# borisfoko/Spark-Text-Clustering

Measured on AMD Instinct MI355X. Metric: LDA E-step docs/sec (node) at k=100, V=2^18; % of HBM roofline, higher is better.
Workload: dtype f64

## Files before the change

### spark-text-clustering_amd/csrc/lda_rows64.hip

```cpp
#include "estep_common.h"
#include "psi64.h"
#include "rows64_layout.h"

#ifndef R64_LOAD_BATCH
#define R64_LOAD_BATCH 3
#endif
#ifndef R64_PRIO
#define R64_PRIO 2
#endif
#ifndef R64_RCP_NR
#define R64_RCP_NR 2
#endif
#ifndef R64_MIRROR
#define R64_MIRROR 1
#endif
#ifndef R64_SB_LDS
#define R64_SB_LDS 0
#endif
#ifndef R64_PSI_TPL
#define R64_PSI_TPL 1
#endif
#ifndef R64_SB_SWZ
#define R64_SB_SWZ 1
#endif
#ifndef R64_PA_LAYOUT
#define R64_PA_LAYOUT 1
#endif
#ifndef R64_LONG_OCC
#define R64_LONG_OCC 1
#endif

namespace stc {
namespace lda {

namespace {

constexpr int kW = 4;
using r64::kPaPitch;
using r64::kSbPitch;
constexpr int kOnChipSets = 6;
constexpr int kMaxSets = 8;

constexpr int kSxPitch = 10;

template <int KL_, int RREG_, int RMAX_>
struct RShape {
  static constexpr int KL = KL_;
  static constexpr int KLP = (KL_ + 1) / 2 * 2;
  static constexpr int KT = 8 * KL_;
  static constexpr int RREG = RREG_;
  static constexpr int RMAX = RMAX_;
  static constexpr int NOVF = RMAX_ > RREG_ ? RMAX_ - RREG_ : 0;
};
template <int KL>
using RCommon = RShape<KL, 5, kOnChipSets>;
template <int KL>
using RLong = RShape<KL, kMaxSets, kMaxSets>;

template <class S>
struct RLds {
  double eth[8][S::KLP] __attribute__((aligned(16)));
  double gam[S::KT];
  double rrow[kW][8 * S::RMAX];
  int rid[kW][8 * S::RMAX];
  double dsum[2];
  double esum[kW] __attribute__((aligned(16)));
  double part[kW][4];
  double cs;
  double apc[S::KT][2] __attribute__((aligned(16)));
  double ac[4] __attribute__((aligned(16)));
  PsiK psik;
  union {
    struct {
      union {
        double pa[8 * S::RMAX][kPaPitch];
        double sx[R64_SB_LDS ? S::KT * kSxPitch : 1] __attribute__((aligned(16)));
      } wv[kW];
      double sb[S::KT][kSbPitch];
    } l;
    double stage[kW][8][S::KT + 2];
  } u __attribute__((aligned(16)));
  double ovf[S::NOVF > 0 ? S::NOVF * kW * S::KL * 64 : 1];
};

struct RDoc {
  int64_t slot, row, mem, s0, e0;
  int nnz, rsets;
  int tid;
  int lane, w, tl, rl;
  int npsi, half, pw, tt, ttl, ttp;
  bool tval, town;
  bool wv;
  int qid;
  double qc, qls, qe2;
#ifdef STC_STAMP
  unsigned long long st0;
#endif
};

template <bool RES>
__device__ __forceinline__ int rows64_tid(const RDoc& d) { return RES ? d.tid : (int)threadIdx.x; }

template <class S, bool STATS, bool BOUND, bool RES, int NPSI>
__device__ __forceinline__ bool rows64_open(const EStepArgs<double>& a, RLds<S>& sm, RDoc& d) {
  const int tid = rows64_tid<RES>(d);
  constexpr int KL = S::KL, KLP = S::KLP;
  const int k = a.k, kp = a.kp;
  const int lane = tid & 63, w = __builtin_amdgcn_readfirstlane(tid >> 6);
  d.lane = lane;
  d.w = w;
  d.tl = lane & 7;
  d.rl = lane >> 3;
  d.npsi = NPSI ? NPSI : (kp > 64 ? 2 : 1);
  d.half = d.npsi == 2 ? (kp + 1) / 2 : kp;
  d.pw = d.npsi == 2 ? (w & 1) : 0;
  d.tt = d.pw * d.half + lane;
  d.tval = lane < d.half && d.tt < kp;
  d.town = lane < d.half && d.tt < k;
  d.ttl = d.tt / KL;
  d.ttp = d.tt - d.ttl * KL;
  const int npsi = d.npsi, tt = d.tt;

  const int qn = 32 * (lane >> 3) + 8 * w + (lane & 7);
  d.wv = lane < 8 * d.rsets && qn < d.nnz;
  const int64_t qe = d.wv ? d.s0 + qn : 0;
  d.qid = d.wv ? a.indices[qe] : 0;
  d.qc = d.wv ? a.values[qe] : 0.0;

  double g0 = 0.0;
  const double alp = d.town ? a.alpha[tt] : 0.0;
  const double pc = d.town ? a.psic[tt] : 0.0;
  if (w < npsi) {
    if (d.tval) {
      sm.apc[tt][0] = alp;
      sm.apc[tt][1] = pc;
    }
    if (d.town) {
      if (a.gamma0) {
        g0 = a.gamma0[d.mem * k + tt];
      } else {
        const uint64_t key = a.key_mode == 0 ? train_doc_key(a.iteration, a.rank, d.mem) : (uint64_t)(a.doc_id_base + d.row);
#ifdef R64_DIAG_NORNG
        g0 = 1.0 + 1e-3 * (double)(key & 1023) + 1e-4 * tt;
#else
        g0 = gamma_sample(doc_stream(a.seed, key), tt, a.gamma_shape);
#endif
      }
    }
    if (d.tval) sm.gam[tt] = g0;
  }
  for (int i = tid; i < 8 * KLP; i += 64 * kW) (&sm.eth[0][0])[i] = 0.0;
  psik_fill(sm.psik, tid, 64 * kW);
  {
    const double gs = wave_sum_d(g0), as = wave_sum_d(alp), cts = wave_sum_d(d.qc);
    if (lane == 0) {
      sm.part[w][0] = w < npsi ? gs : 0.0;
      sm.part[w][1] = w < npsi ? as : 0.0;
      sm.part[w][2] = cts;
    }
  }
  const bool nonempty = __syncthreads_or(d.wv && d.qc != 0.0) != 0;
  const double gsum0 = (sm.part[0][0] + sm.part[1][0]) + (sm.part[2][0] + sm.part[3][0]);
  if (tid == 0) {
    const double asum = (sm.part[0][1] + sm.part[1][1]) + (sm.part[2][1] + sm.part[3][1]);
    const double ctot = (sm.part[0][2] + sm.part[1][2]) + (sm.part[2][2] + sm.part[3][2]);
    sm.ac[0] = asum;
    sm.ac[1] = ctot;
    sm.ac[2] = digamma_fast_d(asum + ctot);
  }

  if (!nonempty) {
    if (w < npsi) {
      if (d.town) {
        if (a.gamma) a.gamma[d.mem * k + tt] = 0.0;
        if (STATS) a.elogth[d.slot * k + tt] = 0.0;
      }
      if (STATS && d.tval) a.eth[d.slot * kp + tt] = 0.0;
    }
    if (tid == 0) {
      if (a.iters) a.iters[d.mem] = 0;
      if (a.nonempty) a.nonempty[d.mem] = 0;
      if (BOUND) a.bound[d.mem] = 0.0;
    }
    return false;
  }
  {
    const double cs0 = digamma_fast_d(gsum0);
    if (w < npsi && d.town) sm.eth[d.ttl][d.ttp] = exp_digamma_minus_v2<R64_RCP_NR>(g0, cs0 + pc);
    if (tid == 0) sm.cs = cs0;
  }
  return true;
}

template <class S, int R, int NPSI>
__device__ __forceinline__ int rows64_iterate(const EStepArgs<double>& a, RLds<S>& sm, RDoc& d, double& qdt) {
  constexpr int KL = S::KL, KLP = S::KLP;
  static_assert(NPSI < 2 || S::KT > 64, "two ψ waves: kp > 64");
  constexpr int RG = R < S::RREG ? R : S::RREG;
  static_assert(R >= 1 && R <= S::RMAX && R - RG <= S::NOVF, "row sets");
  STAMP_DECL
#ifdef STC_STAMP
  st_acc[10] += st_last - d.st0;
#endif
  const int lane = d.lane, w = d.w, tl = d.tl, rl = d.rl;
  const int k = a.k, kp = a.kp, nnz = d.nnz, tt = d.tt, ttl = d.ttl, ttp = d.ttp;
  const int npsi = NPSI ? NPSI : d.npsi, pw = NPSI ? (NPSI == 2 ? (w & 1) : 0) : d.pw;
  const bool town = d.town;
  const int qid = d.qid;
  const double qc = d.qc;
  d.qls = a.logscale[qid];
  const bool mir = R64_MIRROR && npsi == 2;
  double gm = 0.0, em = 0.0;

  double B[RG][KL];
  double* const ovf = sm.ovf + (size_t)w * KL * 64 + lane;
#define BV(j, p) ((j) < RG ? B[(j) < RG ? (j) : 0][p] : ovf[((j) - RG) * kW * KL * 64 + 64 * (p)])
  {
    const int C2 = kp >> 1;
    constexpr int NP = (8 * (S::KT / 2) + 63) / 64;
    double* const stg = &sm.u.stage[w][0][0];
    constexpr int SP = S::KT + 2;
#pragma unroll
    for (int j0 = 0; j0 < R; j0 += R64_LOAD_BATCH) {
      double2 pc[R64_LOAD_BATCH][NP];
#pragma unroll
      for (int jj = 0; jj < R64_LOAD_BATCH; ++jj) {
        const int j = j0 + jj;
        if (j >= R) break;
#pragma unroll
        for (int i = 0; i < NP; ++i) {
          const int c = lane + 64 * i;
          const int srow = c / C2, q = c - srow * C2;
          const int id = __builtin_amdgcn_ds_bpermute((8 * j + (srow & 7)) << 2, qid);
          const bool keep = c < 8 * C2 && 32 * j + 8 * w + srow < nnz;
#ifdef R64_DIAG_NOGATHER
          const double2 x = make_double2(1e-3 * (id & 7), 1e-3 * (q & 7));
#else
          const double2 x = *reinterpret_cast<const double2*>(a.Bp + (int64_t)(keep ? id : 0) * kp + 2 * (keep ? q : 0));
#endif
          pc[jj][i] = keep ? x : make_double2(0.0, 0.0);
        }
      }
#pragma unroll
      for (int jj = 0; jj < R64_LOAD_BATCH; ++jj) {
        const int j = j0 + jj;
        if (j >= R) break;
#pragma unroll
        for (int i = 0; i < NP; ++i) {
          const int c = lane + 64 * i;
          const int srow = c / C2, q = c - srow * C2;
          if (c < 8 * C2) *reinterpret_cast<double2*>(stg + srow * SP + 2 * q) = pc[jj][i];
        }
        __builtin_amdgcn_wave_barrier();
#pragma unroll
        for (int p = 0; p < KL; ++p) {
          const int t = KL * tl + p;
          const double v = t < k ? stg[rl * SP + t] : 0.0;
          if (j < RG) B[j < RG ? j : 0][p] = v;
          else ovf[(j - RG) * kW * KL * 64 + 64 * p] = v;
        }
        __builtin_amdgcn_wave_barrier();
      }
    }
  }

  const double qe2 = d.wv ? fmin(0x1p53 * exp(kLogEps - d.qls), 1e300) : -0x1p53;
  d.qe2 = qe2;
  __syncthreads();
  if (mir && town) {
    gm = sm.gam[tt];
    em = sm.eth[ttl][ttp];
  }

  double* const pa = &sm.u.l.wv[w].pa[0][0];
  int paw_o = 8 * (r64::pa_row(rl, R64_PA_LAYOUT) + tl), par_o = 8 * r64::pa_row(lane, R64_PA_LAYOUT);
#if R64_PA_LAYOUT
  asm volatile("" : "+v"(paw_o), "+v"(par_o));
#endif
  double* const paw = reinterpret_cast<double*>(reinterpret_cast<char*>(pa) + paw_o);
  double* const sb = &sm.u.l.sb[0][0];
  int sbw_o = 8 * r64::sb_slot(KL, tl, 2 * rl, w, R64_SB_SWZ);
  int sp0_o = 8 * (tt * kSbPitch + 2 * r64::sb_read_first(tt, R64_SB_SWZ));
  int sp1_o = 8 * (tt * kSbPitch + 2 * (r64::sb_read_first(tt, R64_SB_SWZ) ^ 1));
#if R64_SB_SWZ
  asm volatile("" : "+v"(sbw_o), "+v"(sp0_o), "+v"(sp1_o));
#endif
  [[maybe_unused]] double* const sbw = reinterpret_cast<double*>(reinterpret_cast<char*>(sb) + sbw_o);
  const double2* const sp0 = reinterpret_cast<const double2*>(reinterpret_cast<const char*>(sb) + sp0_o);
  const double2* const sp1 = reinterpret_cast<const double2*>(reinterpret_cast<const char*>(sb) + sp1_o);
  double* const esw = &sm.esum[w];
  const PsiExpK expk = psi_expk_load(sm.psik);
  double rr[R];
  double qr = 0.0;
  qdt = 0.0;
  double dsum = 0.0;
  int it = 0;
  STAMP(0);
  while (true) {
    {
      double acc[R];
#pragma unroll
      for (int j = 0; j < R; ++j) acc[j] = 0.0;
      constexpr bool OVP = R64_SB_LDS != 0 && R > RG;
      constexpr int NO = OVP ? 2 * (R - RG) : 1;
      double2 en = make_double2(0.0, 0.0);
      double on[NO] = {};
      if constexpr (OVP) {
        en = *reinterpret_cast<const double2*>(&sm.eth[tl][0]);
#pragma unroll
        for (int j = RG; j < R; ++j) {
          on[2 * (j - RG)] = BV(j, 0);
          if (1 < KL) on[2 * (j - RG) + 1] = BV(j, 1);
        }
      }
#pragma unroll
      for (int c = 0; c < KLP / 2; ++c) {
        const double2 e = OVP ? en : *reinterpret_cast<const double2*>(&sm.eth[tl][2 * c]);
        double oc[NO];
#pragma unroll
        for (int i = 0; i < NO; ++i) oc[i] = on[i];
        if (OVP && c + 1 < KLP / 2) {
          en = *reinterpret_cast<const double2*>(&sm.eth[tl][2 * c + 2]);
#pragma unroll
          for (int j = RG; j < R; ++j) {
            on[2 * (j - RG)] = BV(j, 2 * c + 2 < KL ? 2 * c + 2 : 0);
            if (2 * c + 3 < KL) on[2 * (j - RG) + 1] = BV(j, 2 * c + 3 < KL ? 2 * c + 3 : 0);
          }
        }
#pragma unroll
        for (int j = 0; j < R; ++j) {
          const int jo = OVP && j >= RG ? 2 * (j - RG) : 0;
          acc[j] = fma(OVP && j >= RG ? oc[jo] : BV(j, 2 * c), e.x, acc[j]);
          if (2 * c + 1 < KL) acc[j] = fma(OVP && j >= RG ? oc[jo + 1] : BV(j, 2 * c + 1), e.y, acc[j]);
        }
        if (OVP) __builtin_amdgcn_sched_barrier(0);
      }
#pragma unroll
      for (int j = 0; j < R; ++j) paw[8 * kPaPitch * j] = acc[j];
    }
    STAMP(1);
    __builtin_amdgcn_wave_barrier();
    if (R64_PRIO >= 2) __builtin_amdgcn_s_setprio(3);
    if (lane < 8 * R) {
      const double2* const pr = reinterpret_cast<const double2*>(reinterpret_cast<const char*>(pa) + par_o);
      const double2 x0 = pr[0], x1 = pr[1], x2 = pr[2], x3 = pr[3];
      qdt = ((x0.x + x0.y) + (x1.x + x1.y)) + ((x2.x + x2.y) + (x3.x + x3.y));
      const double ph = fma(qe2, 0x1p-53, qdt);
      qr = qc * rcp_nr(ph);
      sm.rrow[w][lane] = qr;
    }
#if R64_PSI_TPL
    const bool live = qe2 >= fma(qe2, 0x1p-53, qdt);
#else
    bool live = false;
    if (lane < 8 * R) live = qe2 >= fma(qe2, 0x1p-53, qdt);
#endif
    if (__builtin_amdgcn_ballot_w64(live) != 0) {
      const double e = wave_sum_d(lane < 8 * R ? qr * (qe2 * 0x1p-53) : 0.0);
      if (lane == 0) *esw = e;
    } else if (lane == 0) {
      *esw = 0.0;
    }
    __builtin_amdgcn_wave_barrier();
#pragma unroll
    for (int j = 0; j < R; ++j) rr[j] = sm.rrow[w][8 * j + rl];
    if (R64_PRIO >= 2) __builtin_amdgcn_s_setprio(0);
    STAMP(2);
    if ((it > 0 && dsum <= a.stop_thr) || it >= a.max_iter) break;

#if R64_SB_LDS
    {
      double* const sx = &sm.u.l.wv[w].sx[0];
      double* const sxw = sx + KL * tl * kSxPitch + rl;
      double ov[R > RG ? R - RG : 1][KL];
#pragma unroll
      for (int j = RG; j < R; ++j) {
#pragma unroll
        for (int p = 0; p < KL; ++p) ov[j - RG][p] = BV(j, p);
      }
#pragma unroll
      for (int p = 0; p < KL; ++p) {
        double acc = 0.0;
#pragma unroll
        for (int j = 0; j < R; ++j) acc = fma(j < RG ? BV(j, p) : ov[j < RG ? 0 : j - RG][p], rr[j], acc);
        sxw[p * kSxPitch] = acc;
      }
      __builtin_amdgcn_wave_barrier();
#pragma unroll
      for (int h = (S::KT - 1) / 64; h >= 0; --h) {
        const int t = lane + 64 * h;
        if (S::KT >= 64 * (h + 1) || t < S::KT) {
          const double2* const xr = reinterpret_cast<const double2*>(sx + t * kSxPitch);
          const double2 x01 = xr[0], x23 = xr[1], x45 = xr[2], x67 = xr[3];
          sb[t * kSbPitch + w] = ((x01.x + x45.x) + (x23.x + x67.x)) + ((x01.y + x45.y) + (x23.y + x67.y));
        }
      }
    }
#else
    {
      double x[16];
#pragma unroll
      for (int p = 0; p < 16; ++p) {
        double acc = 0.0;
        if (p < KL) {
#pragma unroll
          for (int j = 0; j < R; ++j) acc = fma(BV(j, p < KL ? p : 0), rr[j], acc);
        }
        x[p] = acc;
      }
      double s0, s1;
      rs_rows8(x, lane, s0, s1);
      if (2 * rl < KL) sbw[0] = s0;
      if (2 * rl + 1 < KL) sbw[kSbPitch] = s1;
    }
#endif
    STAMP(3);
    __syncthreads();
    STAMP(4);
    const bool psi = npsi == 2 ? ((w >> 1) == (it & 1)) : (w == (it & 3));
    if (psi) {
      if (R64_PRIO >= 1) __builtin_amdgcn_s_setprio(3);
      double dg = 0.0;
      if (town) {
        const double2 x0 = *sp0, x1 = *sp1;
        const double g = mir ? gm : sm.gam[tt], eo = sm.eth[ttl][ttp];
        const double2 ap = *reinterpret_cast<const double2*>(&sm.apc[tt][0]);
        const double2 e01 = *reinterpret_cast<const double2*>(&sm.esum[0]);
        const double2 e23 = *reinterpret_cast<const double2*>(&sm.esum[2]);
        const double s = (x0.x + x0.y) + (x1.x + x1.y);
        const double et = (e01.x + e01.y) + (e23.x + e23.y);
        const double csn = et != 0.0 ? digamma_fast_d(sm.ac[0] + sm.ac[1] - et) : sm.ac[2];
        const double gn = fma(eo, s, ap.x);
        dg = fabs(gn - g);
        sm.gam[tt] = gn;
        const double en = exp_digamma_minus_v4<R64_RCP_NR>(gn, csn + ap.y, expk);
        sm.eth[ttl][ttp] = en;
        gm = gn;
        em = en;
        if (tt == 0) sm.cs = csn;
      }
      if (!mir) {
        const double d = wave_sum_d(dg);
        if (lane == 0) sm.dsum[pw] = d;
      }
      if (R64_PRIO >= 1) __builtin_amdgcn_s_setprio(0);
    } else if (mir) {
      double dg = 0.0;
      if (town) {
        const double al = sm.apc[tt][0];
        const double2 y0 = *sp0, y1 = *sp1;
        const double s = (y0.x + y0.y) + (y1.x + y1.y);
        const double gn = fma(em, s, al);
        dg = fabs(gn - gm);
        gm = gn;
      }
      const double d = wave_sum_d(dg);
      if (lane == 0) sm.dsum[pw] = d;
    }
    STAMP(psi ? 5 : 8);
    __syncthreads();
    dsum = npsi == 2 ? sm.dsum[0] + sm.dsum[1] : sm.dsum[0];
    STAMP(psi ? 6 : 9);
    ++it;
  }
#undef BV
  STAMP_FLUSH
  return it;
}

template <class S, bool STATS, bool BOUND, bool RES>
__device__ __forceinline__ void rows64_close(const EStepArgs<double>& a, RLds<S>& sm, const RDoc& d, int it, double qdt) {
  const int tid = rows64_tid<RES>(d);
  const int lane = d.lane, w = d.w;
  const int k = a.k, kp = a.kp, nnz = d.nnz, npsi = d.npsi, tt = d.tt, ttl = d.ttl, ttp = d.ttp;
  const bool town = d.town, tval = d.tval, wv = d.wv;
  const int64_t slot = d.slot, mem = d.mem, e0 = d.e0;
  const int qid = d.qid;
  const double qc = d.qc, qls = d.qls;
#ifdef STC_STAMP
  const unsigned long long st_close = stamp_now();
#endif
  const double gfin = (w < npsi && town) ? sm.gam[tt] : 0.0;
  {
    const double gs = wave_sum_d(gfin);
    double bt = 0.0, bc = 0.0;
    if (BOUND && wv && qc != 0.0) {
      bt = qc * (log(fmax(qdt, 0x1p-1074)) + qls);
      bc = qc;
    }
    if (BOUND) {
      bt = wave_sum_d(bt);
      bc = wave_sum_d(bc);
    }
    if (lane == 0) {
      sm.part[w][0] = w < npsi ? gs : 0.0;
      sm.part[w][1] = bt;
      sm.part[w][2] = bc;
    }
    if (wv) sm.rid[w][lane] = qid;
  }
  __syncthreads();
  const double gsum = (sm.part[0][0] + sm.part[1][0]) + (sm.part[2][0] + sm.part[3][0]);
  const double psisum = digamma_t<double>(gsum);
  double topic = 0.0;
  if (w < npsi) {
    if (town) {
      const double el = digamma_t<double>(gfin) - psisum;
      if (a.gamma) a.gamma[mem * k + tt] = gfin;
      if (STATS) a.elogth[slot * k + tt] = el;
      if (BOUND) {
        const double alp = sm.apc[tt][0];
        topic = (alp - gfin) * el + (lgamma(gfin) - lgamma(alp));
      }
    }
    if (STATS && tval) a.eth[slot * kp + tt] = sm.eth[ttl][ttp];
  }
  for (int n = tid; n < nnz; n += 64 * kW) {
    const int ws = (n >> 3) & 3, q = 8 * (n >> 5) + (n & 7);
    const double rv = sm.rrow[ws][q];
    a.r[e0 + n] = rv;
    if (STATS && a.keys) {
      a.keys[e0 + n] = (uint32_t)sm.rid[ws][q];
      a.vals[e0 + n] = entry_val<double>(slot, e0 + n, rv);
    }
  }
  if (tid == 0) {
    if (a.iters) a.iters[mem] = it;
    if (a.nonempty) a.nonempty[mem] = 1;
  }
  if (BOUND) {
    topic = wave_sum_d(topic);
    if (lane == 0) sm.part[w][3] = topic;
    __syncthreads();
    if (tid == 0) {
      double tok = 0.0, ctk = 0.0, tp = 0.0;
#pragma unroll
      for (int v = 0; v < kW; ++v) {
        tok += sm.part[v][1];
        ctk += sm.part[v][2];
        tp += sm.part[v][3];
      }
      const double elog_max = sm.cs - psisum;
      a.bound[mem] = tok + ctk * elog_max + tp + (lgamma(sm.ac[0]) - lgamma(gsum));
    }
  }
#ifdef STC_STAMP
  if (lane == 0) atomicAdd(&g_stamps[7], stamp_now() - st_close);
#endif
}

template <class S, bool STATS, bool BOUND, int NPSI, bool LONG, bool RES = LONG>
__device__ __forceinline__ void rows64_doc(const EStepArgs<double>& a, RLds<S>& sm, RDoc& d) {
  d.e0 = a.bptr ? a.bptr[d.slot] : d.s0;
  if (!rows64_open<S, STATS, BOUND, RES, NPSI>(a, sm, d)) return;
  double qdt = 0.0;
  int it;
  if constexpr (LONG) {
    it = d.rsets == 7 ? rows64_iterate<S, 7, NPSI>(a, sm, d, qdt) : rows64_iterate<S, 8, NPSI>(a, sm, d, qdt);
  } else {
    switch (d.rsets) {
      case 1: it = rows64_iterate<S, 1, NPSI>(a, sm, d, qdt); break;
      case 2: it = rows64_iterate<S, 2, NPSI>(a, sm, d, qdt); break;
      case 3: it = rows64_iterate<S, 3, NPSI>(a, sm, d, qdt); break;
      case 4: it = rows64_iterate<S, 4, NPSI>(a, sm, d, qdt); break;
      case 5: it = rows64_iterate<S, 5, NPSI>(a, sm, d, qdt); break;
      default: it = rows64_iterate<S, 6, NPSI>(a, sm, d, qdt); break;
    }
  }
  rows64_close<S, STATS, BOUND, RES>(a, sm, d, it, qdt);
}

template <class S, bool STATS, bool BOUND, int NPSI>
__global__ __launch_bounds__(64 * kW, 2) void k_estep_rows64(EStepArgs<double> a) {
  __shared__ RLds<S> sm;
  if ((int64_t)blockIdx.x >= a.n) return;
  RDoc d;
#ifdef STC_STAMP
  d.st0 = stamp_now();
#endif
  d.slot = a.slot0 + blockIdx.x;
  d.row = a.batch ? (int64_t)a.batch[d.slot] : d.slot;
  d.mem = a.orig ? (int64_t)a.orig[d.slot] : d.slot;
  d.s0 = a.indptr[d.row];
  d.nnz = (int)(a.indptr[d.row + 1] - d.s0);
  d.rsets = (d.nnz + 31) >> 5;
  if (d.rsets > kOnChipSets) return;
  rows64_doc<S, STATS, BOUND, NPSI, false>(a, sm, d);
}

template <class S, bool STATS, bool BOUND, int NPSI>
__global__ __launch_bounds__(64 * kW, 2) void k_estep_rows64_pers(EStepArgs<double> a, int32_t* ticket) {
  __shared__ RLds<S> sm;
  __shared__ int s_tk;
  if (threadIdx.x == 0) s_tk = atomicAdd(ticket, 1);
  __syncthreads();
  int cur = s_tk;
  while (cur < a.n) {
    __syncthreads();
    int nxt = 0;
    if (threadIdx.x == 0) nxt = atomicAdd(ticket, 1);
    RDoc d;
#ifdef STC_STAMP
    d.st0 = stamp_now();
#endif
    d.tid = threadIdx.x;
    asm volatile("" : "+v"(d.tid));
    d.slot = a.slot0 + cur;
    d.row = a.batch ? (int64_t)a.batch[d.slot] : d.slot;
    d.mem = a.orig ? (int64_t)a.orig[d.slot] : d.slot;
    d.s0 = a.indptr[d.row];
    d.nnz = (int)(a.indptr[d.row + 1] - d.s0);
    d.rsets = (d.nnz + 31) >> 5;
    if (d.rsets <= kOnChipSets) rows64_doc<S, STATS, BOUND, NPSI, false, true>(a, sm, d);
    if (threadIdx.x == 0) s_tk = nxt;
    __syncthreads();
    cur = s_tk;
  }
}

__global__ void k_rows64_long_list(EStepArgs<double> a) {
  const int64_t i = (int64_t)blockIdx.x * blockDim.x + threadIdx.x;
  if (i >= a.n) return;
  const int64_t slot = a.slot0 + i;
  const int64_t row = a.batch ? (int64_t)a.batch[slot] : slot;
  const int nnz = (int)(a.indptr[row + 1] - a.indptr[row]);
  if (nnz > 32 * kOnChipSets) a.long_list[1 + atomicAdd(&a.long_list[0], 1)] = (int32_t)i;
}

template <class S, bool STATS, bool BOUND, int NPSI>
__global__ __launch_bounds__(64 * kW, R64_LONG_OCC) void k_estep_rows64_long(EStepArgs<double> a) {
  __shared__ RLds<S> sm;
  const int cnt = a.long_list[0];
  for (int j = blockIdx.x; j < cnt; j += gridDim.x) {
    RDoc d;
#ifdef STC_STAMP
    d.st0 = stamp_now();
#endif
    d.tid = threadIdx.x;
    asm volatile("" : "+v"(d.tid));
    d.slot = a.slot0 + a.long_list[1 + j];
    d.row = a.batch ? (int64_t)a.batch[d.slot] : d.slot;
    d.mem = a.orig ? (int64_t)a.orig[d.slot] : d.slot;
    d.s0 = a.indptr[d.row];
    d.nnz = (int)(a.indptr[d.row + 1] - d.s0);
    d.rsets = (d.nnz + 31) >> 5;
    rows64_doc<S, STATS, BOUND, NPSI, true>(a, sm, d);
    __syncthreads();
  }
}

template <class S, int NPSI>
bool launch_persist(hipStream_t s, const EStepArgs<double>& a, bool stats, bool bound) {
  if (!a.long_list || bound) return false;
  int32_t* ticket = a.long_list + a.n + 1;
  auto go = [&](const void* kern) {
    int dev = 0, cus = 0, per_cu = 0;
    HIP_CHECK(hipGetDevice(&dev));
    HIP_CHECK(hipDeviceGetAttribute(&cus, hipDeviceAttributeMultiprocessorCount, dev));
    HIP_CHECK(hipOccupancyMaxActiveBlocksPerMultiprocessor(&per_cu, kern, 64 * kW, 0));
    if (per_cu < 1) return false;
    HIP_CHECK(hipMemsetAsync(ticket, 0, sizeof(int32_t), s));
    EStepArgs<double> aa = a;
    void* args[] = {&aa, &ticket};
    const int64_t blocks = std::max<int64_t>(1, std::min<int64_t>(a.n, (int64_t)per_cu * cus));
    HIP_CHECK(hipLaunchKernel(kern, dim3((unsigned)blocks), dim3(64 * kW), args, 0, s));
    return true;
  };
  if (stats) return go((const void*)k_estep_rows64_pers<S, true, false, NPSI>);
  return go((const void*)k_estep_rows64_pers<S, false, false, NPSI>);
}
template <class S, int NPSI>
void launch_common(hipStream_t s, const EStepArgs<double>& a, bool stats, bool bound) {
  if (launch_persist<S, NPSI>(s, a, stats, bound)) return;
  const dim3 grid((unsigned)a.n);
  const int threads = 64 * kW;
  if (stats) k_estep_rows64<S, true, false, NPSI><<<grid, threads, 0, s>>>(a);
  else if (bound) k_estep_rows64<S, false, true, NPSI><<<grid, threads, 0, s>>>(a);
  else k_estep_rows64<S, false, false, NPSI><<<grid, threads, 0, s>>>(a);
  KERNEL_CHECK();
}
template <class S, int NPSI>
void launch_long(hipStream_t s, const EStepArgs<double>& a, bool stats, bool bound) {
  if (!a.long_list) throw Error(STC_ERR_STATE, "fp64 rows E-step: no long-document list buffer");
  HIP_CHECK(hipMemsetAsync(a.long_list, 0, sizeof(int32_t), s));
  k_rows64_long_list<<<dim3((unsigned)((a.n + 255) / 256)), 256, 0, s>>>(a);
  KERNEL_CHECK();
  int dev = 0, cus = 0;
  HIP_CHECK(hipGetDevice(&dev));
  HIP_CHECK(hipDeviceGetAttribute(&cus, hipDeviceAttributeMultiprocessorCount, dev));
  const dim3 grid((unsigned)std::max<int64_t>(1, std::min<int64_t>(a.n, (int64_t)cus * R64_LONG_OCC)));
  const int threads = 64 * kW;
  if (stats) k_estep_rows64_long<S, true, false, NPSI><<<grid, threads, 0, s>>>(a);
  else if (bound) k_estep_rows64_long<S, false, true, NPSI><<<grid, threads, 0, s>>>(a);
  else k_estep_rows64_long<S, false, false, NPSI><<<grid, threads, 0, s>>>(a);
  KERNEL_CHECK();
}
template <int KL, int NPSI>
void launch_r(hipStream_t s, const EStepArgs<double>& a, bool stats, bool bound, bool long_docs) {
  if (long_docs) launch_long<RLong<KL>, NPSI>(s, a, stats, bound);
  launch_common<RCommon<KL>, NPSI>(s, a, stats, bound);
}

}

int rows64_row_cap(int k) { return k <= 104 ? 32 * kMaxSets : 0; }
int rows64_onchip_rows(int k) { return k <= 104 ? 32 * kOnChipSets : 0; }

void launch_estep_rows64(hipStream_t s, const EStepArgs<double>& a, bool stats, bool bound, bool long_docs) {
  if (a.n == 0) return;
  if (a.kp > 8 * 13 || a.kp < a.k || (a.kp & 1)) throw Error(STC_ERR_INVALID_ARG, "fp64 rows E-step: bad k / kp");
  constexpr int kOne = R64_PSI_TPL ? 1 : 0, kTwo = R64_PSI_TPL ? 2 : 0;
  if (a.k <= 32) launch_r<4, kOne>(s, a, stats, bound, long_docs);
  else if (a.k <= 56) launch_r<7, kOne>(s, a, stats, bound, long_docs);
  else if (kTwo == 0 || a.kp > 64) launch_r<13, kTwo>(s, a, stats, bound, long_docs);
  else launch_r<13, kOne>(s, a, stats, bound, long_docs);
}

STC_STAMP_READER(stc_debug_stamps_rows64)

}
}
```

### spark-text-clustering_amd/csrc/psi64.h

```cpp
#pragma once

#include "estep_common.h"

namespace stc {
namespace lda {
namespace psi64 {

__device__ __forceinline__ double fma_s(double a, double b, double c) {
  double d;
  asm("v_fma_f64 %0, %1, %2, %3" : "=v"(d) : "v"(a), "v"(b), "s"(c));
  return d;
}
__device__ __forceinline__ double fma_sb(double a, double b, double c) {
  double d;
  asm("v_fma_f64 %0, %1, %2, %3" : "=v"(d) : "v"(a), "s"(b), "v"(c));
  return d;
}
__device__ __forceinline__ double mul_s(double a, double b) {
  double d;
  asm("v_mul_f64 %0, %1, %2" : "=v"(d) : "v"(a), "s"(b));
  return d;
}
__device__ __forceinline__ double add_s(double a, double b) {
  double d;
  asm("v_add_f64 %0, %1, %2" : "=v"(d) : "v"(a), "s"(b));
  return d;
}
__device__ __forceinline__ double sub_s(double b, double a) {
  double d;
  asm("v_add_f64 %0, -%1, %2" : "=v"(d) : "v"(a), "s"(b));
  return d;
}
typedef float pkf2 __attribute__((ext_vector_type(2)));
__device__ __forceinline__ double trunc_fix_pk(double f6, double xs) {
  const double nb = floor(sub_s(5.0, xs)) + 1.0;
  const float rb = __builtin_amdgcn_rcpf((float)xs + (float)nb);
  const pkf2 u = {(float)f6, rb * rb};
  pkf2 a = u * (pkf2)(-12318.55039822477f) + (pkf2)(2372.137971404805f);
  a = a * u + (pkf2)(-260.94994774566294f);
  a = a * u + (pkf2)(26.284421368293753f);
  a = a * u + (pkf2)(-3.053401198888146f);
  const pkf2 u2 = u * u, u4 = u2 * u2, u8 = u4 * u4;
  const pkf2 e = (u8 * u) * a;
  return (double)(e.x - e.y);
}
template <int RCP_STEPS>
__device__ __forceinline__ double rcp_n(double q) {
  double r = __builtin_amdgcn_rcp(q);
#pragma unroll
  for (int i = 0; i < RCP_STEPS; ++i) r = fma(r, fma(-q, r, 1.0), r);
  return r;
}
template <int RCP_STEPS>
__device__ __forceinline__ double exp_digamma_minus_v2(double x, double cst) {
  const bool sh = x <= 5.0;
  const double xs = sh ? x : 1.0;
  const double u = xs * add_s(xs, 5.0);
  const double num = fma_s(add_s(mul_s(u, 3.0), 20.0), u, 24.0) * fma(xs, 2.0, 5.0);
  const double den = u * fma_s(add_s(u, 10.0), u, 24.0);
  const double iq = rcp_n<RCP_STEPS>(den);
  double c = num * iq;
  c = fma(fma(-den, c, num), iq, c);
  const double y = sh ? add_s(x, 6.0) : x;
  const double iy = rcp_n<RCP_STEPS>(y);
  const double f = iy * iy;
  double t = add_s(mul_s(f, 3617.0 / 8160.0), -1.0 / 12.0);
  t = fma_s(t, f, 691.0 / 32760.0);
  t = fma_s(t, f, -1.0 / 132.0);
  t = fma_s(t, f, 1.0 / 240.0);
  t = fma_s(t, f, -1.0 / 252.0);
  t = fma_s(t, f, 1.0 / 120.0);
  t = fma_s(t, f, -1.0 / 12.0) * f;
  const double shift = sh ? trunc_fix_pk(f, xs) - c : 0.0;
  const double z = (fma(-0.5, iy, shift) + t) - cst;
  const double n = __builtin_rint(mul_s(z, 1.4426950408889634));
  double r = fma_sb(n, -6.93147180369123816490e-01, z);
  r = fma_sb(n, -1.90821492927058770002e-10, r);
  const double r2 = r * r;
  double e = add_s(mul_s(r2, 1.0 / 479001600.0), 1.0 / 3628800.0);
  e = fma_s(e, r2, 1.0 / 40320.0);
  e = fma_s(e, r2, 1.0 / 720.0);
  e = fma_s(e, r2, 1.0 / 24.0);
  e = fma(e, r2, 0.5);
  e = fma(e, r2, 1.0);
  double o = add_s(mul_s(r2, 1.0 / 6227020800.0), 1.0 / 39916800.0);
  o = fma_s(o, r2, 1.0 / 362880.0);
  o = fma_s(o, r2, 1.0 / 5040.0);
  o = fma_s(o, r2, 1.0 / 120.0);
  o = fma_s(o, r2, 1.0 / 6.0);
  o = fma(o, r2, 1.0);
  const double ez = __builtin_ldexp(fma(r, o, e), (int)fmax(n, -1100.0));
  return y * ez;
}

enum PsiKSlot {
  PK_LOG2E, PK_LN2HI, PK_LN2LO,
  PK_E0, PK_E1, PK_E2, PK_E3, PK_E4,
  PK_O0, PK_O1, PK_O2, PK_O3, PK_O5,
  PK_O4,
  PK_N
};
struct alignas(16) PsiK {
  double k[(PK_N + 1) / 2 * 2];
};
__device__ __forceinline__ void psik_fill(PsiK& t, int tid, int nthr) {
  const double v[PK_N] = {1.4426950408889634, -6.93147180369123816490e-01, -1.90821492927058770002e-10,
                          1.0 / 479001600.0, 1.0 / 3628800.0, 1.0 / 40320.0, 1.0 / 720.0, 1.0 / 24.0,
                          1.0 / 6227020800.0, 1.0 / 39916800.0, 1.0 / 362880.0, 1.0 / 5040.0, 1.0 / 120.0,
                          1.0 / 6.0};
  for (int i = tid; i < PK_N; i += nthr) t.k[i] = v[i];
}
struct PsiExpK {
  double log2e, ln2hi, ln2lo, e0, e1, e2, e3, e4, o0, o1, o2, o3, o5, o4;
};
__device__ __forceinline__ PsiExpK psi_expk_load(const PsiK& T) {
  const double* K = T.k;
  PsiExpK c{K[PK_LOG2E], K[PK_LN2HI], K[PK_LN2LO], K[PK_E0], K[PK_E1], K[PK_E2], K[PK_E3], K[PK_E4],
            K[PK_O0],    K[PK_O1],    K[PK_O2],    K[PK_O3], K[PK_O5], K[PK_O4]};
  asm volatile("" : "+v"(c.log2e), "+v"(c.ln2hi), "+v"(c.ln2lo), "+v"(c.e0), "+v"(c.e1), "+v"(c.e2), "+v"(c.e3));
  asm volatile("" : "+v"(c.e4), "+v"(c.o0), "+v"(c.o1), "+v"(c.o2), "+v"(c.o3), "+v"(c.o5), "+v"(c.o4));
  return c;
}
__device__ __forceinline__ double exp_vk(double z, const PsiExpK& C) {
#pragma clang fp contract(off)
  const double n = __builtin_rint(z * C.log2e);
  double r = __builtin_fma(n, C.ln2hi, z);
  r = __builtin_fma(n, C.ln2lo, r);
  const double r2 = r * r;
  double e = r2 * C.e0 + C.e1;
  e = __builtin_fma(e, r2, C.e2);
  e = __builtin_fma(e, r2, C.e3);
  e = __builtin_fma(e, r2, C.e4);
  e = __builtin_fma(e, r2, 0.5);
  e = __builtin_fma(e, r2, 1.0);
  double o = r2 * C.o0 + C.o1;
  o = __builtin_fma(o, r2, C.o2);
  o = __builtin_fma(o, r2, C.o3);
  o = __builtin_fma(o, r2, C.o5);
  o = __builtin_fma(o, r2, C.o4);
  o = __builtin_fma(o, r2, 1.0);
  return __builtin_ldexp(__builtin_fma(r, o, e), (int)fmax(n, -1100.0));
}
template <int RCP_STEPS>
__device__ __forceinline__ double exp_digamma_minus_v4(double x, double cst, const PsiExpK& C) {
  const bool sh = x <= 5.0;
  const double xs = sh ? x : 1.0;
  const double u = xs * add_s(xs, 5.0);
  const double num = fma_s(add_s(mul_s(u, 3.0), 20.0), u, 24.0) * fma(xs, 2.0, 5.0);
  const double den = u * fma_s(add_s(u, 10.0), u, 24.0);
  const double iq = rcp_n<RCP_STEPS>(den);
  double c = num * iq;
  c = fma(fma(-den, c, num), iq, c);
  const double y = sh ? add_s(x, 6.0) : x;
  const double iy = rcp_n<RCP_STEPS>(y);
  const double f = iy * iy;
  double t = add_s(mul_s(f, 3617.0 / 8160.0), -1.0 / 12.0);
  t = fma_s(t, f, 691.0 / 32760.0);
  t = fma_s(t, f, -1.0 / 132.0);
  t = fma_s(t, f, 1.0 / 240.0);
  t = fma_s(t, f, -1.0 / 252.0);
  t = fma_s(t, f, 1.0 / 120.0);
  t = fma_s(t, f, -1.0 / 12.0) * f;
  const double shift = sh ? trunc_fix_pk(f, xs) - c : 0.0;
  const double z = (fma(-0.5, iy, shift) + t) - cst;
  return y * exp_vk(z, C);
}

}
using psi64::exp_digamma_minus_v2;
using psi64::PsiK;
using psi64::psik_fill;
using psi64::PsiExpK;
using psi64::psi_expk_load;
using psi64::exp_digamma_minus_v4;
}
}
```

Before: 1.824 million.

## Defer dsum read, reorder psi update ahead of esum, skip redundant esum stores

Reads the convergence sums from shared memory during the next matvec instead of right after the second barrier, which takes an LDS load off the post-barrier critical path. The psi update now computes the digamma part before reading esum, and moves the rare correction behind an unlikely branch. The esum write is skipped when it was already zero on the previous iteration. An eager mode hoists x+6 and trunc_fix inside the psi polynomial, and lane-0 tests are made opaque to the compiler. These reorderings raise register pressure and add branch logic to a tight per-iteration loop.

```diff
diff --git a/spark-text-clustering_amd/csrc/lda_rows64.hip b/spark-text-clustering_amd/csrc/lda_rows64.hip
--- a/spark-text-clustering_amd/csrc/lda_rows64.hip
+++ b/spark-text-clustering_amd/csrc/lda_rows64.hip
@@ -25,6 +25,18 @@
 #endif
 #ifndef R64_PA_LAYOUT
 #define R64_PA_LAYOUT 1
+#endif
+#ifndef R64_DSUM_LATE
+#define R64_DSUM_LATE 1
+#endif
+#ifndef R64_PSI_FIRST
+#define R64_PSI_FIRST 1
+#endif
+#ifndef R64_PSI_EAGER
+#define R64_PSI_EAGER 1
+#endif
+#ifndef R64_WORKER_LINE
+#define R64_WORKER_LINE 1
 #endif
 #ifndef R64_LONG_OCC
 #define R64_LONG_OCC 1
@@ -294,6 +306,8 @@
   double qr = 0.0;
   qdt = 0.0;
   double dsum = 0.0;
+  [[maybe_unused]] double ds0 = 0.0, ds1 = 0.0;
+  [[maybe_unused]] uint32_t esnz = 1;
   int it = 0;
   STAMP(0);
   while (true) {
@@ -335,12 +349,38 @@
         }
         if (OVP) __builtin_amdgcn_sched_barrier(0);
       }
+#if R64_DSUM_LATE
+      ds0 = sm.dsum[0];
+      if (npsi == 2) ds1 = sm.dsum[1];
+#endif
 #pragma unroll
       for (int j = 0; j < R; ++j) paw[8 * kPaPitch * j] = acc[j];
     }
     STAMP(1);
     __builtin_amdgcn_wave_barrier();
     if (R64_PRIO >= 2) __builtin_amdgcn_s_setprio(3);
+#if R64_WORKER_LINE
+    {
+      double ph = -1.0;
+      if (lane < 8 * R) {
+        const double2* const pr = reinterpret_cast<const double2*>(reinterpret_cast<const char*>(pa) + par_o);
+        const double2 x0 = pr[0], x1 = pr[1], x2 = pr[2], x3 = pr[3];
+        qdt = ((x0.x + x0.y) + (x1.x + x1.y)) + ((x2.x + x2.y) + (x3.x + x3.y));
+        ph = fma(qe2, 0x1p-53, qdt);
+        qr = qc * rcp_nr(ph);
+        sm.rrow[w][lane] = qr;
+      }
+      const uint64_t vm = __builtin_amdgcn_ballot_w64(qe2 >= ph);
+      if (__builtin_expect(((uint32_t)vm | (uint32_t)(vm >> 32) | esnz) != 0, 0)) {
+        double e = 0.0;
+        if (vm != 0) e = wave_sum_d(lane < 8 * R ? qr * (qe2 * 0x1p-53) : 0.0);
+        int l0 = lane;
+        asm volatile("" : "+v"(l0));
+        if (l0 == 0) *esw = e;
+        esnz = __builtin_amdgcn_readfirstlane(vm != 0);
+      }
+    }
+#else
     if (lane < 8 * R) {
       const double2* const pr = reinterpret_cast<const double2*>(reinterpret_cast<const char*>(pa) + par_o);
       const double2 x0 = pr[0], x1 = pr[1], x2 = pr[2], x3 = pr[3];
@@ -361,12 +401,18 @@
     } else if (lane == 0) {
       *esw = 0.0;
     }
+#endif
     __builtin_amdgcn_wave_barrier();
 #pragma unroll
     for (int j = 0; j < R; ++j) rr[j] = sm.rrow[w][8 * j + rl];
     if (R64_PRIO >= 2) __builtin_amdgcn_s_setprio(0);
     STAMP(2);
+#if R64_DSUM_LATE
+    dsum = npsi == 2 ? ds0 + ds1 : ds0;
+    if (((int)(it > 0) & (int)(dsum <= a.stop_thr)) | (int)(it >= a.max_iter)) break;
+#else
     if ((it > 0 && dsum <= a.stop_thr) || it >= a.max_iter) break;
+#endif
 
 #if R64_SB_LDS
     {
@@ -427,13 +473,28 @@
         const double2 ap = *reinterpret_cast<const double2*>(&sm.apc[tt][0]);
         const double2 e01 = *reinterpret_cast<const double2*>(&sm.esum[0]);
         const double2 e23 = *reinterpret_cast<const double2*>(&sm.esum[2]);
+#if R64_PSI_FIRST
+        const double cflat = sm.ac[2];
+        const double s = (x0.x + x0.y) + (x1.x + x1.y);
+        const double gn = fma(eo, s, ap.x);
+        dg = fabs(gn - g);
+        sm.gam[tt] = gn;
+        double y;
+        const double zt = psi_part_v4<R64_RCP_NR, R64_PSI_EAGER != 0>(gn, y);
+        __builtin_amdgcn_sched_barrier(0);
+        const double et = (e01.x + e01.y) + (e23.x + e23.y);
+        double csn = cflat;
+        if (__builtin_expect(et != 0.0, 0)) [[clang::always_inline]] csn = digamma_fast_d(sm.ac[0] + sm.ac[1] - et);
+        const double en = y * exp_vk(zt - (csn + ap.y), expk);
+#else
         const double s = (x0.x + x0.y) + (x1.x + x1.y);
         const double et = (e01.x + e01.y) + (e23.x + e23.y);
         const double csn = et != 0.0 ? digamma_fast_d(sm.ac[0] + sm.ac[1] - et) : sm.ac[2];
         const double gn = fma(eo, s, ap.x);
         dg = fabs(gn - g);
         sm.gam[tt] = gn;
-        const double en = exp_digamma_minus_v4<R64_RCP_NR>(gn, csn + ap.y, expk);
+        const double en = exp_digamma_minus_v4<R64_RCP_NR, R64_PSI_EAGER != 0>(gn, csn + ap.y, expk);
+#endif
         sm.eth[ttl][ttp] = en;
         gm = gn;
         em = en;
@@ -455,11 +516,19 @@
         gm = gn;
       }
       const double d = wave_sum_d(dg);
+#if R64_WORKER_LINE
+      int l0 = lane;
+      asm volatile("" : "+v"(l0));
+      if (l0 == 0) sm.dsum[pw] = d;
+#else
       if (lane == 0) sm.dsum[pw] = d;
+#endif
     }
     STAMP(psi ? 5 : 8);
     __syncthreads();
+#if !R64_DSUM_LATE
     dsum = npsi == 2 ? sm.dsum[0] + sm.dsum[1] : sm.dsum[0];
+#endif
     STAMP(psi ? 6 : 9);
     ++it;
   }
diff --git a/spark-text-clustering_amd/csrc/psi64.h b/spark-text-clustering_amd/csrc/psi64.h
--- a/spark-text-clustering_amd/csrc/psi64.h
+++ b/spark-text-clustering_amd/csrc/psi64.h
@@ -141,8 +141,8 @@
   o = __builtin_fma(o, r2, 1.0);
   return __builtin_ldexp(__builtin_fma(r, o, e), (int)fmax(n, -1100.0));
 }
-template <int RCP_STEPS>
-__device__ __forceinline__ double exp_digamma_minus_v4(double x, double cst, const PsiExpK& C) {
+template <int RCP_STEPS, bool EAGER>
+__device__ __forceinline__ double psi_part_v4(double x, double& y_out) {
   const bool sh = x <= 5.0;
   const double xs = sh ? x : 1.0;
   const double u = xs * add_s(xs, 5.0);
@@ -151,9 +151,19 @@
   const double iq = rcp_n<RCP_STEPS>(den);
   double c = num * iq;
   c = fma(fma(-den, c, num), iq, c);
-  const double y = sh ? add_s(x, 6.0) : x;
+  double x6 = 0.0;
+  if (EAGER) {
+    x6 = add_s(x, 6.0);
+    asm volatile("" : "+v"(x6));
+  }
+  const double y = sh ? (EAGER ? x6 : add_s(x, 6.0)) : x;
   const double iy = rcp_n<RCP_STEPS>(y);
   const double f = iy * iy;
+  double tf = 0.0;
+  if (EAGER) {
+    tf = trunc_fix_pk(f, xs);
+    asm volatile("" : "+v"(c), "+v"(tf));
+  }
   double t = add_s(mul_s(f, 3617.0 / 8160.0), -1.0 / 12.0);
   t = fma_s(t, f, 691.0 / 32760.0);
   t = fma_s(t, f, -1.0 / 132.0);
@@ -161,8 +171,14 @@
   t = fma_s(t, f, -1.0 / 252.0);
   t = fma_s(t, f, 1.0 / 120.0);
   t = fma_s(t, f, -1.0 / 12.0) * f;
-  const double shift = sh ? trunc_fix_pk(f, xs) - c : 0.0;
-  const double z = (fma(-0.5, iy, shift) + t) - cst;
+  const double shift = sh ? (EAGER ? tf : trunc_fix_pk(f, xs)) - c : 0.0;
+  y_out = y;
+  return fma(-0.5, iy, shift) + t;
+}
+template <int RCP_STEPS, bool EAGER = false>
+__device__ __forceinline__ double exp_digamma_minus_v4(double x, double cst, const PsiExpK& C) {
+  double y;
+  const double z = psi_part_v4<RCP_STEPS, EAGER>(x, y) - cst;
   return y * exp_vk(z, C);
 }
 
@@ -173,5 +189,7 @@
 using psi64::PsiExpK;
 using psi64::psi_expk_load;
 using psi64::exp_digamma_minus_v4;
+using psi64::psi_part_v4;
+using psi64::exp_vk;
 }
 }
```

Result: faster. 1.896 million, median of 6 (+3.9%).
